# jerinphilip/whisper.tflite

Measured on AMD Instinct MI355X. Metric: audio-sec/s (RTF) whisper-tiny 30s clips batch=32 at 1/2/4/8 MI355X, higher is better.
Workload: dtype f32 (operands as two fp16 planes, f16 MFMA, f32 accumulate); 1 GPU; whisper-tiny batch=32x30s synthetic mel U(-1,1.5), fp32, random-init weights (BASELINE.json configs[1]); mel resident in HBM -> token ids on host; clips_per_gpu=32, global_batch=32, decoder_positions=30, argmax_steps=27, parallelism=clip-parallel dp1, one RCCL all_gather of id records per 8 batches, pipelined=True, batches_in_flight=10, decoder=2 consecutive steps' batches share one decoder chain (dec_pair, dec_group), last_batches_announced=2, priming_batches=1

## Files before the change

whisper.tflite_amd/csrc/k_gemm_planes.hip:

```cpp
#include <hip/hip_runtime.h>

#include <algorithm>
#include <cstdlib>
#include <cstring>
#include <type_traits>

#include "bf16_split.h"
#include "kernels.h"

namespace wt {

static int g_plane_gemm_mode = -1;
int plane_gemm_mode() {
  if (g_plane_gemm_mode < 0) {
    const char* v = getenv("WT_PLANE_GEMM_MODE");
    g_plane_gemm_mode = v ? atoi(v) : 2;
  }
  return g_plane_gemm_mode;
}
void set_plane_gemm_mode(int m) { g_plane_gemm_mode = m; }

namespace {

using f32x16 = __attribute__((ext_vector_type(16))) float;
using f32x4 = __attribute__((ext_vector_type(4))) float;
using half8 = __attribute__((ext_vector_type(8))) _Float16;
using half4 = __attribute__((ext_vector_type(4))) _Float16;
using u32x4 = __attribute__((ext_vector_type(4))) unsigned;

constexpr int BK = 32;

struct PlaneGemmDev {
  const _Float16* A;
  long a_plane;
  const _Float16* W;
  float* C;
  _Float16* P;
  long p_plane;
  const float* bias;
  const float* R;
  const float* pos;
  int M, N, K;
  int a_rpb;
  long a_bs;
  int lda;
  int c_rpb;
  long c_bs;
  int ldc;
  int pos_period;
  int kv_batch, kv_heads, kv_dmodel;
  float descale;
  float out_scale[3];
  int seg;
  const float* ln_g;
  const float* ln_b;
  _Float16* ln_P;
  long ln_plane;
  float ln_scale;
  float* ln_y32;
  int* nonfinite;
};

__host__ __device__ __forceinline__ constexpr int chunk_swizzle(int row) { return (0 - (row >> 2)) & 3; }

template <int QA, int QW, int NW, int QPW>
__device__ __forceinline__ void setup_stage_dma(const PlaneGemmDev& g, int m0, int n0, int wid, int lane, unsigned (&voff)[QPW],
                                                const unsigned char* (&ubase)[QPW], unsigned (&kstep)[QPW]) {
  const int srow = lane >> 2;
  const int nkt = g.K / BK;
#pragma unroll
  for (int j = 0; j < QPW; ++j) {
    const int q = wid + NW * j;
    if (q < 2 * QA) {
      const bool lo = q >= QA;
      const int row = 16 * (lo ? q - QA : q) + srow;
      const int chunk = (lane & 3) ^ chunk_swizzle(row);
      int m = m0 + row;
      m = m < g.M ? m : g.M - 1;
      voff[j] = (unsigned)(2 * ((lo ? g.a_plane : 0) + (long)(m / g.a_rpb) * g.a_bs + (long)(m % g.a_rpb) * g.lda + chunk * 8));
      ubase[j] = reinterpret_cast<const unsigned char*>(g.A);
      kstep[j] = BK * 2;
    } else {
      const int wq = q - 2 * QA;
      const int rg = wq % QW, plane = wq / QW;
      voff[j] = (unsigned)(lane * 16);
      ubase[j] = reinterpret_cast<const unsigned char*>(g.W) + ((size_t)(n0 / 16 + rg) * nkt * 2 + plane) * 1024;
      kstep[j] = 2048;
    }
  }
}

template <int MI_, int NI_>
struct Acc32 {
  static constexpr int MI = MI_, NI = NI_;
  f32x16 t[MI_][NI_];
  __device__ __forceinline__ void zero() {
#pragma unroll
    for (int i = 0; i < MI_; ++i)
#pragma unroll
      for (int j = 0; j < NI_; ++j)
#pragma unroll
        for (int r = 0; r < 16; ++r) t[i][j][r] = 0.0f;
  }
  __device__ __forceinline__ float get(int mi, int ni, int i) const { return t[mi][ni][i]; }
  __device__ __forceinline__ void set(int mi, int ni, int i, float v) { t[mi][ni][i] = v; }
  __device__ __forceinline__ void stage_write(int mi, int ni, float* stage, int lane, float scale) const {
    const int l31 = lane & 31, lh = lane >> 5;
#pragma unroll
    for (int r = 0; r < 16; ++r) stage[((r & 3) + 8 * (r >> 2) + 4 * lh) * 32 + (l31 ^ (lh * 20))] = t[mi][ni][r] * scale;
  }
};
template <int MI_, int NI_>
struct Acc16 {
  static constexpr int MI = MI_, NI = NI_;
  f32x4 t[2 * MI_][2 * NI_];
  __device__ __forceinline__ void zero() {
#pragma unroll
    for (int i = 0; i < 2 * MI_; ++i)
#pragma unroll
      for (int j = 0; j < 2 * NI_; ++j)
#pragma unroll
        for (int r = 0; r < 4; ++r) t[i][j][r] = 0.0f;
  }
  __device__ __forceinline__ float get(int mi, int ni, int i) const { return t[2 * mi + (i >> 3)][2 * ni + ((i >> 2) & 1)][i & 3]; }
  __device__ __forceinline__ void set(int mi, int ni, int i, float v) { t[2 * mi + (i >> 3)][2 * ni + ((i >> 2) & 1)][i & 3] = v; }
  __device__ __forceinline__ void stage_write(int mi, int ni, float* stage, int lane, float scale) const {
    const int c = lane & 15, q = lane >> 4;
#pragma unroll
    for (int a = 0; a < 2; ++a)
#pragma unroll
      for (int b = 0; b < 2; ++b)
#pragma unroll
        for (int r = 0; r < 4; ++r)
          stage[(16 * a + 4 * q + r) * 32 + ((16 * b + c) ^ ((q & 1) * 20))] = t[2 * mi + a][2 * ni + b][r] * scale;
  }
};

struct NoEpilogueHook {
  static constexpr bool active = false;
  __device__ __forceinline__ void operator()() const {}
};
template <class F>
struct ActiveEpilogueHook {
  static constexpr bool active = true;
  F& f;
  __device__ __forceinline__ void operator()() const { f(); }
};
template <int EPI, bool PLANES_OUT, int WN, bool LN, class Acc, class Hook = NoEpilogueHook>
__device__ __forceinline__ void planes_epilogue(const PlaneGemmDev& g, Acc& acc, unsigned char* smem, int m0, int n0, int wid, int wm,
                                                int wn, int lane, Hook hook = Hook{}) {
  constexpr int MI = Acc::MI, NI = Acc::NI;
  constexpr int BN = WN * NI * 32, NW = 2 * WN, BM = 64 * MI;
  __syncthreads();

  constexpr int SLD = 32;
  float* const stage = reinterpret_cast<float*>(smem) + wid * (32 * SLD);
  constexpr int CPL = PLANES_OUT ? 8 : 4;
  constexpr int LPR = 32 / CPL;
  constexpr int RPS = 64 / LPR;
  const int prow = lane / LPR, c0 = (lane % LPR) * CPL;
  float bias_all[NI][CPL];
#pragma unroll
  for (int ni = 0; ni < NI; ++ni)
#pragma unroll
    for (int e = 0; e < CPL; ++e) bias_all[ni][e] = (EPI & kEpiBias) ? g.bias[n0 + (wn * NI + ni) * 32 + c0 + e] : 0.0f;
  if constexpr (Hook::active) {
#pragma unroll
    for (int ni = 0; ni < NI; ++ni)
#pragma unroll
      for (int e = 0; e < CPL; e += 4)
        asm volatile("" : "+v"(bias_all[ni][e]), "+v"(bias_all[ni][e + 1]), "+v"(bias_all[ni][e + 2]), "+v"(bias_all[ni][e + 3]));
    hook();
  }
#pragma unroll
  for (int ni = 0; ni < NI; ++ni) {
    const int n = n0 + (wn * NI + ni) * 32 + c0;
    float bias_v[CPL];
#pragma unroll
    for (int e = 0; e < CPL; ++e) bias_v[e] = bias_all[ni][e];
    const float oscale = PLANES_OUT ? g.out_scale[n / g.seg] : 1.0f;
    const int slab = (EPI & kEpiKvLayout) ? n / g.kv_dmodel : 0, rem = (EPI & kEpiKvLayout) ? n % g.kv_dmodel : 0;
    const int head = rem >> 6, dd = rem & 63;
#pragma unroll
    for (int mi = 0; mi < MI; ++mi) {
      acc.stage_write(mi, ni, stage, lane, g.descale);
      const int mbase = m0 + wm * (32 * MI) + mi * 32;
      const int mb0 = mbase / g.c_rpb, mt0 = mbase % g.c_rpb;
      const int mp0 = (EPI & kEpiPos) ? mbase % g.pos_period : 0;
#pragma unroll
      for (int p = 0; p < 32 / RPS; ++p) {
        const int row = p * RPS + prow;
        float v[CPL];
#pragma unroll
        for (int e = 0; e < CPL; e += 4) {
          const f32x4 t = *reinterpret_cast<const f32x4*>(&stage[row * SLD + ((c0 + e) ^ (((row >> 2) & 1) * 20))]);
          v[e] = t[0], v[e + 1] = t[1], v[e + 2] = t[2], v[e + 3] = t[3];
        }
        if (mbase + row < g.M) {
          int mb = mb0, mt = mt0 + row;
          if (mt >= g.c_rpb) mt -= g.c_rpb, mb += 1;
#pragma unroll
          for (int e = 0; e < CPL; e += 2) {
            v[e] += bias_v[e];
            v[e + 1] += bias_v[e + 1];
            if (EPI & kEpiGelu) {
              const f32x2_t gl = gelu_erf2(f32x2_t{v[e], v[e + 1]});
              v[e] = gl[0];
              v[e + 1] = gl[1];
            }
          }
          if (EPI & kEpiPos) {
            int mp = mp0 + row;
            if (mp >= g.pos_period) mp -= g.pos_period;
#pragma unroll
            for (int e = 0; e < CPL; e += 4) {
              const f32x4 t = *reinterpret_cast<const f32x4*>(g.pos + (long)mp * g.N + n + e);
              v[e] += t[0], v[e + 1] += t[1], v[e + 2] += t[2], v[e + 3] += t[3];
            }
          }
          if (PLANES_OUT) {
            const long o = (long)mb * g.c_bs + (long)mt * g.ldc + n;
            u32x4 hi, lo;
#pragma unroll
            for (int e = 0; e < CPL; e += 2) {
              unsigned h, l;
              split_f16x2(v[e] * oscale, v[e + 1] * oscale, &h, &l);
              hi[e / 2] = h;
              lo[e / 2] = l;
            }
            *reinterpret_cast<u32x4*>(g.P + o) = hi;
            *reinterpret_cast<u32x4*>(g.P + g.p_plane + o) = lo;
          } else if (EPI & kEpiKvLayout) {
            const long o = (((long)slab * g.kv_batch + mb) * g.kv_heads + head) * (long)g.c_rpb * 64 + (long)mt * 64 + dd;
            __builtin_nontemporal_store(f32x4{v[0], v[1], v[2], v[3]}, reinterpret_cast<f32x4*>(g.C + o));
          } else if constexpr ((EPI & kEpiPower) != 0) {
            using f32x2 = __attribute__((ext_vector_type(2))) float;
            const long o = (long)mb * g.c_bs + (long)mt * g.ldc + (n >> 1);
            *reinterpret_cast<f32x2*>(g.C + o) = f32x2{v[0] * v[0] + v[1] * v[1], v[2] * v[2] + v[3] * v[3]};
          } else {
            const long o = (long)mb * g.c_bs + (long)mt * g.ldc + n;
            f32x4 out = {v[0], v[1], v[2], v[3]};
            if (EPI & kEpiResidual) out += *reinterpret_cast<const f32x4*>(g.R + o);
            *reinterpret_cast<f32x4*>(g.C + o) = out;
            if constexpr (LN) {
#pragma unroll
              for (int e = 0; e < 4; ++e) acc.set(mi, ni, 4 * p + e, out[e]);
            }
          }
        } else if constexpr (LN) {
#pragma unroll
          for (int e = 0; e < 4; ++e) acc.set(mi, ni, 4 * p + e, 0.0f);
        }
      }
    }
  }
  if constexpr (LN) {
    float* const part = reinterpret_cast<float*>(smem) + NW * (32 * SLD);
    const int rbase = wm * (32 * MI) + prow;
    float mean[MI][4], rstd[MI][4];
#pragma unroll
    for (int pass = 0; pass < 2; ++pass) {
#pragma unroll
      for (int mi = 0; mi < MI; ++mi)
#pragma unroll
        for (int p = 0; p < 4; ++p) {
          float t = 0.0f;
#pragma unroll
          for (int ni = 0; ni < NI; ++ni)
#pragma unroll
            for (int e = 0; e < 4; ++e) {
              const float x = acc.get(mi, ni, 4 * p + e) - (pass ? mean[mi][p] : 0.0f);
              t += pass ? x * x : x;
            }
          t += __shfl_xor(t, 1, 64);
          t += __shfl_xor(t, 2, 64);
          t += __shfl_xor(t, 4, 64);
          if ((lane & 7) == 0) part[pass * (BM * 4) + (rbase + mi * 32 + p * 8) * 4 + wn] = t;
        }
      __syncthreads();
#pragma unroll
      for (int mi = 0; mi < MI; ++mi)
#pragma unroll
        for (int p = 0; p < 4; ++p) {
          const f32x4 q = *reinterpret_cast<const f32x4*>(&part[pass * (BM * 4) + (rbase + mi * 32 + p * 8) * 4]);
          const float tot = ((q[0] + q[1]) + (q[2] + q[3])) * (1.0f / (float)BN);
          if (pass == 0) {
            mean[mi][p] = tot;
          } else {
            if (g.nonfinite != nullptr && (lane & 7) == 0 && wn == 0 && !(fabsf(mean[mi][p]) <= 3.0e38f && tot <= 3.0e38f)) atomicOr(g.nonfinite, 1);
            rstd[mi][p] = rsqrtf(tot + 1e-5f);
          }
        }
    }
#pragma unroll
    for (int ni = 0; ni < NI; ++ni) {
      const int n = n0 + (wn * NI + ni) * 32 + c0;
      const f32x4 gg = *reinterpret_cast<const f32x4*>(g.ln_g + n), bb = *reinterpret_cast<const f32x4*>(g.ln_b + n);
#pragma unroll
      for (int mi = 0; mi < MI; ++mi)
#pragma unroll
        for (int p = 0; p < 4; ++p) {
          const int m = m0 + rbase + mi * 32 + p * 8;
          if (m >= g.M) continue;
          f32x4 y;
#pragma unroll
          for (int e = 0; e < 4; ++e) y[e] = (acc.get(mi, ni, 4 * p + e) - mean[mi][p]) * rstd[mi][p] * gg[e] + bb[e];
          const long o = (long)m * BN + n;
          if (g.ln_y32 != nullptr) __builtin_nontemporal_store(y, reinterpret_cast<f32x4*>(g.ln_y32 + o));
          unsigned h0, l0, h1, l1;
          split_f16x2(y[0] * g.ln_scale, y[1] * g.ln_scale, &h0, &l0);
          split_f16x2(y[2] * g.ln_scale, y[3] * g.ln_scale, &h1, &l1);
          using u32x2 = __attribute__((ext_vector_type(2))) unsigned;
          *reinterpret_cast<u32x2*>(g.ln_P + o) = u32x2{h0, h1};
          *reinterpret_cast<u32x2*>(g.ln_P + g.ln_plane + o) = u32x2{l0, l1};
        }
    }
  }
}

template <int EPI, bool PLANES_OUT, int WN, int NI, int MI, bool LN = false>
__global__ __launch_bounds__(128 * WN, WN == 2 ? 2 : 2) void gemm_planes_tile(PlaneGemmDev g) {
  static_assert(!LN || (!PLANES_OUT && WN == 4 && NI == 3), "LayerNorm fusion: fp32 output, 384-column tile");
  constexpr int BN = WN * NI * 32, NW = 2 * WN, BM = 64 * MI;
  constexpr int kAPlane = BM * BK * 2, kWPlane = BN * BK * 2;
  constexpr int kStage = 2 * kAPlane + 2 * kWPlane;
  constexpr int QA = BM / 16, QW = BN / 16;
  constexpr int QT = 2 * QA + 2 * QW, QPW = QT / NW;
  static_assert(QT % NW == 0, "whole instructions per wavefront");
  extern __shared__ __attribute__((aligned(16))) unsigned char smem[];

  const int nb = gridDim.x, bid = blockIdx.x;
  const int q8 = nb >> 3, r8 = nb & 7, xcd = bid & 7;
  const int logical = (xcd < r8 ? xcd * (q8 + 1) : r8 * (q8 + 1) + (xcd - r8) * q8) + (bid >> 3);
  const int n_tiles = g.N / BN;
  const int m0 = (logical / n_tiles) * BM;
  const int n0 = (logical % n_tiles) * BN;

  const int tid = threadIdx.x;
  const int lane = tid & 63, wid = __builtin_amdgcn_readfirstlane(tid >> 6);
  const int wm = wid / WN, wn = wid % WN;
  const int l31 = lane & 31, lh = lane >> 5;

  unsigned voff[QPW], kstep[QPW];
  const unsigned char* ubase[QPW];
  const unsigned lds_base = (unsigned)(size_t)(const __attribute__((address_space(3))) unsigned char*)smem;
  setup_stage_dma<QA, QW, NW, QPW>(g, m0, n0, wid, lane, voff, ubase, kstep);
  auto issue_stage = [&](int kt, int buf) {
#pragma unroll
    for (int j = 0; j < QPW; ++j) {
      const unsigned long long sb = reinterpret_cast<unsigned long long>(ubase[j]) + (size_t)kt * kstep[j];
      const unsigned dst = lds_base + (unsigned)(buf * kStage + (wid + NW * j) * 1024);
      lds_dma16_sgpr(voff[j], sb, dst);
    }
  };

  Acc32<MI, NI> accs;
  accs.zero();
  auto& acc = accs.t;

  const int swz = chunk_swizzle(l31);
  const int a_off = (wm * (32 * MI) + l31) * 64, b_off = 2 * kAPlane + (wn * NI * 32 + l31) * 64;
  auto compute = [&](int buf) {
    const unsigned char* base = smem + buf * kStage;
#pragma unroll
    for (int ks = 0; ks < BK / 16; ++ks) {
      const int slot = ((ks * 2 + lh) ^ swz) * 16;
      half8 ah[MI], al[MI], bh[NI], bl[NI];
#pragma unroll
      for (int i = 0; i < MI; ++i) {
        ah[i] = *reinterpret_cast<const half8*>(base + a_off + i * 32 * 64 + slot);
        al[i] = *reinterpret_cast<const half8*>(base + kAPlane + a_off + i * 32 * 64 + slot);
      }
#pragma unroll
      for (int j = 0; j < NI; ++j) {
        bh[j] = *reinterpret_cast<const half8*>(base + b_off + j * 32 * 64 + slot);
        bl[j] = *reinterpret_cast<const half8*>(base + kWPlane + b_off + j * 32 * 64 + slot);
      }
#pragma unroll
      for (int i = 0; i < MI; ++i)
#pragma unroll
        for (int j = 0; j < NI; ++j) acc[i][j] = __builtin_amdgcn_mfma_f32_32x32x16_f16(ah[i], bl[j], acc[i][j], 0, 0, 0);
#pragma unroll
      for (int i = 0; i < MI; ++i)
#pragma unroll
        for (int j = 0; j < NI; ++j) acc[i][j] = __builtin_amdgcn_mfma_f32_32x32x16_f16(al[i], bh[j], acc[i][j], 0, 0, 0);
#pragma unroll
      for (int i = 0; i < MI; ++i)
#pragma unroll
        for (int j = 0; j < NI; ++j) acc[i][j] = __builtin_amdgcn_mfma_f32_32x32x16_f16(ah[i], bh[j], acc[i][j], 0, 0, 0);
    }
  };

  const int nkt = g.K / BK;
  issue_stage(0, 0);
  for (int kt = 0; kt < nkt; ++kt) {
    asm volatile("s_waitcnt vmcnt(0)" ::: "memory");
    __builtin_amdgcn_s_barrier();
    if (kt + 1 < nkt) issue_stage(kt + 1, (kt + 1) & 1);
    compute(kt & 1);
  }
  planes_epilogue<EPI, PLANES_OUT, WN, LN>(g, accs, smem, m0, n0, wid, wm, wn, lane);
}

#ifdef WT_PP_STAMPS
__device__ long long g_pp_stamps[1024 * 8 * 9];
#define PP_STAMP(i)                                  \
  do {                                               \
    const long long t_ = __builtin_readcyclecounter(); \
    st_[i] += t_ - tl_;                              \
    tl_ = t_;                                        \
  } while (0)
#else
#define PP_STAMP(i) \
  do {              \
  } while (0)
#endif

template <int EPI, bool PLANES_OUT, int MI, bool LN = false>
__global__ __launch_bounds__(512, 2) void gemm_planes_pp(PlaneGemmDev g) {
  constexpr int WN = 4, NI = 3;
  static_assert(!LN || !PLANES_OUT, "LayerNorm fusion: fp32 output");
  constexpr int BN = WN * NI * 32, NW = 2 * WN, BM = 64 * MI;
  constexpr int kAPlane = BM * BK * 2, kWPlane = BN * BK * 2;
  constexpr int kStage = 2 * kAPlane + 2 * kWPlane;
  constexpr int QA = BM / 16, QW = BN / 16;
  constexpr int QT = 2 * QA + 2 * QW, QPW = QT / NW;
  static_assert(QT % NW == 0, "whole instructions per wavefront");
#ifdef WT_PP_STAMPS
  const long long t_kernel_ = __builtin_readcyclecounter();
  const long long r_kernel_ = (long long)__builtin_amdgcn_s_memrealtime();
#endif
  extern __shared__ __attribute__((aligned(16))) unsigned char smem[];

  const int nb = gridDim.x, bid = blockIdx.x;
  const int q8 = nb >> 3, r8 = nb & 7, xcd = bid & 7;
  const int logical = (xcd < r8 ? xcd * (q8 + 1) : r8 * (q8 + 1) + (xcd - r8) * q8) + (bid >> 3);
  const int n_tiles = g.N / BN;
  const int m0 = (logical / n_tiles) * BM;
  const int n0 = (logical % n_tiles) * BN;

  const int tid = threadIdx.x;
  const int lane = tid & 63, wid = __builtin_amdgcn_readfirstlane(tid >> 6);
  const int wm = wid / WN, wn = wid % WN;
  const int l31 = lane & 31, lh = lane >> 5;

  unsigned voff[QPW], kstep[QPW];
  const unsigned char* ubase[QPW];
  const unsigned lds_base = (unsigned)(size_t)(const __attribute__((address_space(3))) unsigned char*)smem;
  setup_stage_dma<QA, QW, NW, QPW>(g, m0, n0, wid, lane, voff, ubase, kstep);
  auto issue_stage = [&](int kt, int buf) {
#pragma unroll
    for (int j = 0; j < QPW; ++j) {
      const unsigned long long sb = reinterpret_cast<unsigned long long>(ubase[j]) + (size_t)kt * kstep[j];
      const unsigned dst = lds_base + (unsigned)(buf * kStage + (wid + NW * j) * 1024);
      lds_dma16_sgpr(voff[j], sb, dst);
    }
  };

  Acc32<MI, NI> accs;
  accs.zero();
  auto& acc = accs.t;

  const int swz = chunk_swizzle(l31);
  const int a_off = (wm * (32 * MI) + l31) * 64, b_off = 2 * kAPlane + (wn * NI * 32 + l31) * 64;
  half8 ah[MI], al[MI], bh[NI], bl[NI];
  auto load_frags = [&](int buf, int ks) {
    const unsigned char* base = smem + buf * kStage;
    const int slot = ((ks * 2 + lh) ^ swz) * 16;
#pragma unroll
    for (int i = 0; i < MI; ++i) {
      ah[i] = *reinterpret_cast<const half8*>(base + a_off + i * 32 * 64 + slot);
      al[i] = *reinterpret_cast<const half8*>(base + kAPlane + a_off + i * 32 * 64 + slot);
    }
#pragma unroll
    for (int j = 0; j < NI; ++j) {
      bh[j] = *reinterpret_cast<const half8*>(base + b_off + j * 32 * 64 + slot);
      bl[j] = *reinterpret_cast<const half8*>(base + kWPlane + b_off + j * 32 * 64 + slot);
    }
  };
  auto compute = [&]() {
#pragma unroll
    for (int i = 0; i < MI; ++i)
#pragma unroll
      for (int j = 0; j < NI; ++j) acc[i][j] = __builtin_amdgcn_mfma_f32_32x32x16_f16(ah[i], bl[j], acc[i][j], 0, 0, 0);
#pragma unroll
    for (int i = 0; i < MI; ++i)
#pragma unroll
      for (int j = 0; j < NI; ++j) acc[i][j] = __builtin_amdgcn_mfma_f32_32x32x16_f16(al[i], bh[j], acc[i][j], 0, 0, 0);
#pragma unroll
    for (int i = 0; i < MI; ++i)
#pragma unroll
      for (int j = 0; j < NI; ++j) acc[i][j] = __builtin_amdgcn_mfma_f32_32x32x16_f16(ah[i], bh[j], acc[i][j], 0, 0, 0);
  };
  auto phase_end = [&]() {
    __builtin_amdgcn_sched_barrier(0);
    __builtin_amdgcn_s_barrier();
    __builtin_amdgcn_sched_barrier(0);
  };
  auto reads_done = [&]() { asm volatile("s_waitcnt lgkmcnt(0)" ::: "memory"); };
  auto dma_done = [&]() { asm volatile("s_waitcnt vmcnt(0)" ::: "memory"); };

  const int nkt = g.K / BK;
  issue_stage(0, 0);
  if (nkt > 1) {
    issue_stage(1, 1);
    asm volatile("s_waitcnt vmcnt(%0)" ::"n"(QPW) : "memory");
  } else {
    dma_done();
  }
  phase_end();
  if (wm == 1) phase_end();
  load_frags(0, 0);
  reads_done();
  phase_end();
#ifdef WT_PP_STAMPS
  long long st_[9] = {0, 0, 0, 0, 0, 0, 0, 0, 0};
  long long tl_ = __builtin_readcyclecounter();
  const long long t_begin_ = tl_;
  st_[5] = tl_ - t_kernel_;
#endif
  for (int kt = 0; kt < nkt; ++kt) {
    compute();
    phase_end();
    PP_STAMP(0);
    load_frags(kt & 1, 1);
    reads_done();
    if (wm == 1) dma_done();
    phase_end();
    PP_STAMP(1);
    compute();
    if (wm == 0) dma_done();
    phase_end();
    PP_STAMP(2);
    if (kt + 1 < nkt) {
      if (kt + 2 < nkt) issue_stage(kt + 2, kt & 1);
      load_frags((kt + 1) & 1, 0);
      reads_done();
    }
    phase_end();
    PP_STAMP(3);
  }
  if (wm == 0) phase_end();
#ifdef WT_PP_STAMPS
  const long long t_loop_end_ = __builtin_readcyclecounter();
  st_[4] = t_loop_end_ - t_begin_;
#endif
  planes_epilogue<EPI, PLANES_OUT, WN, LN>(g, accs, smem, m0, n0, wid, wm, wn, lane);
#ifdef WT_PP_STAMPS
  {
    const long long t_end_ = __builtin_readcyclecounter();
    st_[6] = t_end_ - t_loop_end_;
    st_[7] = t_end_ - t_kernel_;
    st_[8] = (long long)__builtin_amdgcn_s_memrealtime() - r_kernel_;
    if (lane == 0 && blockIdx.x < 1024)
      for (int i = 0; i < 9; ++i) g_pp_stamps[(blockIdx.x * 8 + wid) * 9 + i] = st_[i];
  }
#endif
}

template <int EPI, bool PLANES_OUT, bool LN = false>
__global__ __launch_bounds__(512, 2) void gemm_planes_pp16(PlaneGemmDev g) {
  constexpr int WN = 4, NI = 3, MI = 3;
  static_assert(!LN || !PLANES_OUT, "LayerNorm fusion: fp32 output");
  constexpr int BN = WN * NI * 32, NW = 2 * WN, BM = 64 * MI;
  constexpr int kAPlane = BM * BK * 2, kWPlane = BN * BK * 2;
  constexpr int kStage = 2 * kAPlane + 2 * kWPlane;
  constexpr int QA = BM / 16, QW = BN / 16;
  constexpr int QT = 2 * QA + 2 * QW, QPW = QT / NW;
  static_assert(QT % NW == 0, "whole instructions per wavefront");
#ifdef WT_PP_STAMPS
  const long long t_kernel_ = __builtin_readcyclecounter();
  const long long r_kernel_ = (long long)__builtin_amdgcn_s_memrealtime();
#endif
  extern __shared__ __attribute__((aligned(16))) unsigned char smem[];

  const int nb = gridDim.x, bid = blockIdx.x;
  const int q8 = nb >> 3, r8 = nb & 7, xcd = bid & 7;
  const int logical = (xcd < r8 ? xcd * (q8 + 1) : r8 * (q8 + 1) + (xcd - r8) * q8) + (bid >> 3);
  const int n_tiles = g.N / BN;
  const int m0 = (logical / n_tiles) * BM;
  const int n0 = (logical % n_tiles) * BN;

  const int tid = threadIdx.x;
  const int lane = tid & 63, wid = __builtin_amdgcn_readfirstlane(tid >> 6);
  const int wm = wid / WN, wn = wid % WN;

  unsigned voff[QPW], kstep[QPW];
  const unsigned char* ubase[QPW];
  const unsigned lds_base = (unsigned)(size_t)(const __attribute__((address_space(3))) unsigned char*)smem;
  setup_stage_dma<QA, QW, NW, QPW>(g, m0, n0, wid, lane, voff, ubase, kstep);
  auto issue_stage = [&](int kt, int buf) {
#pragma unroll
    for (int j = 0; j < QPW; ++j) {
      const unsigned long long sb = reinterpret_cast<unsigned long long>(ubase[j]) + (size_t)kt * kstep[j];
      const unsigned dst = lds_base + (unsigned)(buf * kStage + (wid + NW * j) * 1024);
      lds_dma16_sgpr(voff[j], sb, dst);
    }
  };

  Acc16<MI, NI> accs;
  accs.zero();
  auto& acc = accs.t;

  const int fc = lane & 15, fq = lane >> 4;
  const int frag = fc * 64 + ((fq ^ chunk_swizzle(fc)) * 16);
  const int a_off = wm * (32 * MI) * 64 + frag, b_off = 2 * kAPlane + wn * (NI * 32) * 64 + frag;
  half8 ah[3], al[3], bh[6], bl[6];
  auto load_b = [&](int buf) {
    const unsigned char* base = smem + buf * kStage + b_off;
#pragma unroll
    for (int j = 0; j < 6; ++j) {
      bh[j] = *reinterpret_cast<const half8*>(base + j * 1024);
      bl[j] = *reinterpret_cast<const half8*>(base + kWPlane + j * 1024);
    }
  };
  auto load_a = [&](int buf, int half) {
    const unsigned char* base = smem + buf * kStage + a_off + half * 3 * 1024;
#pragma unroll
    for (int i = 0; i < 3; ++i) {
      ah[i] = *reinterpret_cast<const half8*>(base + i * 1024);
      al[i] = *reinterpret_cast<const half8*>(base + kAPlane + i * 1024);
    }
  };
  auto compute = [&](auto half_c) {
    constexpr int H = decltype(half_c)::value;
#pragma unroll
    for (int i = 0; i < 3; ++i)
#pragma unroll
      for (int j = 0; j < 6; ++j) acc[3 * H + i][j] = __builtin_amdgcn_mfma_f32_16x16x32_f16(ah[i], bl[j], acc[3 * H + i][j], 0, 0, 0);
#pragma unroll
    for (int i = 0; i < 3; ++i)
#pragma unroll
      for (int j = 0; j < 6; ++j) acc[3 * H + i][j] = __builtin_amdgcn_mfma_f32_16x16x32_f16(al[i], bh[j], acc[3 * H + i][j], 0, 0, 0);
#pragma unroll
    for (int i = 0; i < 3; ++i)
#pragma unroll
      for (int j = 0; j < 6; ++j) acc[3 * H + i][j] = __builtin_amdgcn_mfma_f32_16x16x32_f16(ah[i], bh[j], acc[3 * H + i][j], 0, 0, 0);
  };
  using H0 = std::integral_constant<int, 0>;
  using H1 = std::integral_constant<int, 1>;
  auto phase_end = [&]() {
    __builtin_amdgcn_sched_barrier(0);
    __builtin_amdgcn_s_barrier();
    __builtin_amdgcn_sched_barrier(0);
  };
  auto reads_done = [&]() { asm volatile("s_waitcnt lgkmcnt(0)" ::: "memory"); };
  auto dma_done = [&]() { asm volatile("s_waitcnt vmcnt(0)" ::: "memory"); };

  const int nkt = g.K / BK;
  issue_stage(0, 0);
  if (nkt > 1) {
    issue_stage(1, 1);
    asm volatile("s_waitcnt vmcnt(%0)" ::"n"(QPW) : "memory");
  } else {
    dma_done();
  }
  phase_end();
  if (wm == 1) phase_end();
  load_b(0);
  load_a(0, 0);
  reads_done();
  phase_end();
#ifdef WT_PP_STAMPS
  long long st_[9] = {0, 0, 0, 0, 0, 0, 0, 0, 0};
  long long tl_ = __builtin_readcyclecounter();
  const long long t_begin_ = tl_;
  st_[5] = tl_ - t_kernel_;
#endif
  for (int kt = 0; kt < nkt; ++kt) {
    compute(H0{});
    phase_end();
    PP_STAMP(0);
    load_a(kt & 1, 1);
    reads_done();
    if (wm == 1) dma_done();
    phase_end();
    PP_STAMP(1);
    compute(H1{});
    if (wm == 0) dma_done();
    phase_end();
    PP_STAMP(2);
    if (kt + 1 < nkt) {
      if (kt + 2 < nkt) issue_stage(kt + 2, kt & 1);
      load_b((kt + 1) & 1);
      load_a((kt + 1) & 1, 0);
      reads_done();
    }
    phase_end();
    PP_STAMP(3);
  }
  if (wm == 0) phase_end();
#ifdef WT_PP_STAMPS
  const long long t_loop_end_ = __builtin_readcyclecounter();
  st_[4] = t_loop_end_ - t_begin_;
#endif
  planes_epilogue<EPI, PLANES_OUT, WN, LN>(g, accs, smem, m0, n0, wid, wm, wn, lane);
#ifdef WT_PP_STAMPS
  {
    const long long t_end_ = __builtin_readcyclecounter();
    st_[6] = t_end_ - t_loop_end_;
    st_[7] = t_end_ - t_kernel_;
    st_[8] = (long long)__builtin_amdgcn_s_memrealtime() - r_kernel_;
    if (lane == 0 && blockIdx.x < 1024)
      for (int i = 0; i < 9; ++i) g_pp_stamps[(blockIdx.x * 8 + wid) * 9 + i] = st_[i];
  }
#endif
}

template <int EPI>
__global__ __launch_bounds__(512, 2) void gemm_planes_pp16_persist(PlaneGemmDev g, int total_tiles) {
  constexpr int WN = 4, NI = 3, MI = 3;
  constexpr bool PLANES_OUT = true;
  static_assert((EPI & ~(kEpiBias | kEpiGelu)) == 0, "bias / GELU epilogues with plane output");
  constexpr int BN = WN * NI * 32, NW = 2 * WN, BM = 64 * MI;
  constexpr int kAPlane = BM * BK * 2, kWPlane = BN * BK * 2;
  constexpr int kStage = 2 * kAPlane + 2 * kWPlane;
  constexpr int QA = BM / 16, QW = BN / 16;
  constexpr int QT = 2 * QA + 2 * QW, QPW = QT / NW;
  constexpr int kEpiStores = MI * NI * 4;
  extern __shared__ __attribute__((aligned(16))) unsigned char smem[];

  const int grid = gridDim.x, bid = blockIdx.x;
  const int q8 = total_tiles >> 3, r8 = total_tiles & 7;
  const int n_tiles = g.N / BN;
  const int tid = threadIdx.x;
  const int lane = tid & 63, wid = __builtin_amdgcn_readfirstlane(tid >> 6);
  const int wm = wid / WN, wn = wid % WN;

  unsigned voff[QPW], kstep[QPW];
  const unsigned char* ubase[QPW];
  const unsigned lds_base = (unsigned)(size_t)(const __attribute__((address_space(3))) unsigned char*)smem;
  int m0 = 0, n0 = 0;
  auto set_tile = [&](int vid) {
    const int xcd = vid & 7;
    const int logical = (xcd < r8 ? xcd * (q8 + 1) : r8 * (q8 + 1) + (xcd - r8) * q8) + (vid >> 3);
    m0 = (logical / n_tiles) * BM;
    n0 = (logical % n_tiles) * BN;
    setup_stage_dma<QA, QW, NW, QPW>(g, m0, n0, wid, lane, voff, ubase, kstep);
  };
  auto issue_stage = [&](int kt) {
    const int buf = (kt + 1) & 1;
#pragma unroll
    for (int j = 0; j < QPW; ++j) {
      const unsigned long long sb = reinterpret_cast<unsigned long long>(ubase[j]) + (size_t)kt * kstep[j];
      lds_dma16_sgpr(voff[j], sb, lds_base + (unsigned)(buf * kStage + (wid + NW * j) * 1024));
    }
  };

  Acc16<MI, NI> accs;
  auto& acc = accs.t;
  const int fc = lane & 15, fq = lane >> 4;
  const int frag = fc * 64 + ((fq ^ chunk_swizzle(fc)) * 16);
  const int a_off = wm * (32 * MI) * 64 + frag, b_off = 2 * kAPlane + wn * (NI * 32) * 64 + frag;
  half8 ah[3], al[3], bh[6], bl[6];
  auto load_b = [&](int kt) {
    const unsigned char* base = smem + ((kt + 1) & 1) * kStage + b_off;
#pragma unroll
    for (int j = 0; j < 6; ++j) {
      bh[j] = *reinterpret_cast<const half8*>(base + j * 1024);
      bl[j] = *reinterpret_cast<const half8*>(base + kWPlane + j * 1024);
    }
  };
  auto load_a = [&](int kt, int half) {
    const unsigned char* base = smem + ((kt + 1) & 1) * kStage + a_off + half * 3 * 1024;
#pragma unroll
    for (int i = 0; i < 3; ++i) {
      ah[i] = *reinterpret_cast<const half8*>(base + i * 1024);
      al[i] = *reinterpret_cast<const half8*>(base + kAPlane + i * 1024);
    }
  };
  auto compute = [&](auto half_c) {
    constexpr int H = decltype(half_c)::value;
#pragma unroll
    for (int i = 0; i < 3; ++i)
#pragma unroll
      for (int j = 0; j < 6; ++j) acc[3 * H + i][j] = __builtin_amdgcn_mfma_f32_16x16x32_f16(ah[i], bl[j], acc[3 * H + i][j], 0, 0, 0);
#pragma unroll
    for (int i = 0; i < 3; ++i)
#pragma unroll
      for (int j = 0; j < 6; ++j) acc[3 * H + i][j] = __builtin_amdgcn_mfma_f32_16x16x32_f16(al[i], bh[j], acc[3 * H + i][j], 0, 0, 0);
#pragma unroll
    for (int i = 0; i < 3; ++i)
#pragma unroll
      for (int j = 0; j < 6; ++j) acc[3 * H + i][j] = __builtin_amdgcn_mfma_f32_16x16x32_f16(ah[i], bh[j], acc[3 * H + i][j], 0, 0, 0);
  };
  using H0 = std::integral_constant<int, 0>;
  using H1 = std::integral_constant<int, 1>;
  auto phase_end = [&]() {
    __builtin_amdgcn_sched_barrier(0);
    __builtin_amdgcn_s_barrier();
    __builtin_amdgcn_sched_barrier(0);
  };
  auto reads_done = [&]() { asm volatile("s_waitcnt lgkmcnt(0)" ::: "memory"); };
  auto dma_done = [&]() { asm volatile("s_waitcnt vmcnt(0)" ::: "memory"); };

  const int nkt = g.K / BK;
  int vid = bid;
  set_tile(vid);
  issue_stage(0);
  issue_stage(1);
  asm volatile("s_waitcnt vmcnt(%0)" ::"n"(QPW) : "memory");
  phase_end();
  for (;;) {
    if (wm == 1) phase_end();
    accs.zero();
    load_b(0);
    load_a(0, 0);
    reads_done();
    phase_end();
    for (int kt = 0; kt < nkt; ++kt) {
      compute(H0{});
      phase_end();
      load_a(kt, 1);
      reads_done();
      if (wm == 1) dma_done();
      phase_end();
      compute(H1{});
      if (wm == 0) dma_done();
      phase_end();
      if (kt + 1 < nkt) {
        if (kt + 2 < nkt) issue_stage(kt + 2);
        load_b(kt + 1);
        load_a(kt + 1, 0);
        reads_done();
      }
      phase_end();
    }
    if (wm == 0) phase_end();
    const int m_cur = m0, n_cur = n0;
    const int next = vid + grid;
    const bool has_next = next < total_tiles;
    const bool whole = m_cur + BM <= g.M;
    auto prefetch = [&]() {
      if (has_next) {
        set_tile(next);
        issue_stage(0);
      }
    };
    planes_epilogue<EPI, PLANES_OUT, WN, false>(g, accs, smem, m_cur, n_cur, wid, wm, wn, lane, ActiveEpilogueHook<decltype(prefetch)>{prefetch});
    if (!has_next) break;
    if (whole) {
      asm volatile("s_waitcnt vmcnt(%0)" ::"n"(kEpiStores) : "memory");
    } else {
      dma_done();
    }
    phase_end();
    issue_stage(1);
    vid = next;
  }
}

template <int EPI, bool PLANES_OUT, int WN, int NI, int MI = 3, bool LN = false>
void launch_planes_shape(const PlaneGemmDev& g, hipStream_t s, int n_cu = 0) {
  constexpr int BN = WN * NI * 32, BM = 64 * MI;
  const int blocks = ((g.M + BM - 1) / BM) * (g.N / BN);
  constexpr size_t smem = 2 * (2 * BM * BK * 2 + 2 * BN * BK * 2);
  static const bool raised = [] {
    (void)hipFuncSetAttribute(reinterpret_cast<const void*>(&gemm_planes_tile<EPI, PLANES_OUT, WN, NI, MI, LN>),
                              hipFuncAttributeMaxDynamicSharedMemorySize, 160 * 1024);
    return true;
  }();
  (void)raised;
  if constexpr (WN == 4 && NI == 3 && MI == 3) {
    if constexpr (PLANES_OUT && !LN && (EPI & ~(kEpiBias | kEpiGelu)) == 0) {
      const int cu = n_cu > 0 ? n_cu : 256;
      if (plane_gemm_mode() == 2 && cu % 8 == 0 && blocks >= 2 * cu && (g.K / BK) % 2 == 0 && g.K / BK >= 4) {
        static const bool raised_p = [] {
          (void)hipFuncSetAttribute(reinterpret_cast<const void*>(&gemm_planes_pp16_persist<EPI>), hipFuncAttributeMaxDynamicSharedMemorySize,
                                    160 * 1024);
          return true;
        }();
        (void)raised_p;
        WT_LAUNCH_TIMED((gemm_planes_pp16_persist<EPI>), dim3(cu), dim3(512), smem, s, g, blocks);
        return;
      }
    }
    if (plane_gemm_mode() == 2 || plane_gemm_mode() == 4) {
      static const bool raised_pp16 = [] {
        (void)hipFuncSetAttribute(reinterpret_cast<const void*>(&gemm_planes_pp16<EPI, PLANES_OUT, LN>),
                                  hipFuncAttributeMaxDynamicSharedMemorySize, 160 * 1024);
        return true;
      }();
      (void)raised_pp16;
      WT_LAUNCH_TIMED((gemm_planes_pp16<EPI, PLANES_OUT, LN>), dim3(blocks), dim3(512), smem, s, g);
      return;
    }
    if (plane_gemm_mode() == 1) {
      static const bool raised_pp = [] {
        (void)hipFuncSetAttribute(reinterpret_cast<const void*>(&gemm_planes_pp<EPI, PLANES_OUT, MI, LN>),
                                  hipFuncAttributeMaxDynamicSharedMemorySize, 160 * 1024);
        return true;
      }();
      (void)raised_pp;
      WT_LAUNCH_TIMED((gemm_planes_pp<EPI, PLANES_OUT, MI, LN>), dim3(blocks), dim3(512), smem, s, g);
      return;
    }
  }
  WT_LAUNCH_TIMED((gemm_planes_tile<EPI, PLANES_OUT, WN, NI, MI, LN>), dim3(blocks), dim3(128 * WN), smem, s, g);
}

template <int EPI, bool PLANES_OUT>
bool launch_planes(const PlaneGemmDev& g, int n_cu, hipStream_t s) {
  static const int forced = [] {
    const char* v = getenv("WT_PLANE_TILE");
    return v ? atoi(v) : 0;
  }();
  const int cu = n_cu > 0 ? n_cu : 256;
  auto rounds = [&](long tiles) { return (tiles + cu - 1) / cu; };
  const long rt192 = (g.M + 191) / 192, rt256 = (g.M + 255) / 256;
  const bool can_wide = g.N % 384 == 0;
  const double c_wide = can_wide ? 192.0 * 3 * rounds(rt192 * (g.N / 384)) : 1e30;
  const double c_tall = can_wide ? 256.0 * 3 * 1.08 * rounds(rt256 * (g.N / 384)) : 1e30;
  const double c_narrow = 192.0 * 1.1 * rounds(rt192 * (g.N / 128));
  int pick = c_wide <= c_narrow ? (c_tall < c_wide ? 2 : 1) : (c_tall < c_narrow ? 2 : 0);
  if (forced == 128) pick = 0;
  if (forced == 384 && can_wide) pick = 1;
  if (forced == 256 && can_wide) pick = 2;
  if constexpr (!PLANES_OUT && (EPI == (kEpiBias | kEpiResidual) || EPI == (kEpiBias | kEpiGelu | kEpiPos))) {
    if (g.ln_P != nullptr && g.N == 384 && pick != 0) {
      if (pick == 2) {
        launch_planes_shape<EPI, false, 4, 3, 4, true>(g, s);
      } else {
        launch_planes_shape<EPI, false, 4, 3, 3, true>(g, s);
      }
      return true;
    }
  }
  if (pick == 2) {
    launch_planes_shape<EPI, PLANES_OUT, 4, 3, 4>(g, s);
  } else if (pick == 1) {
    launch_planes_shape<EPI, PLANES_OUT, 4, 3, 3>(g, s, n_cu);
  } else {
    launch_planes_shape<EPI, PLANES_OUT, 2, 2, 3>(g, s);
  }
  return false;
}

}

std::vector<unsigned short> split_weight_planes(const float* W, int N, int K, int Kpad, float scale) {
  if (N % 16 != 0 || Kpad % 32 != 0 || K > Kpad) throw Error(kErrInvalidArg, "split_weight_planes: N % 16, Kpad % 32");
  std::vector<unsigned short> out(size_t(2) * N * Kpad, 0);
  const int nkt = Kpad / 32;
  for (int n = 0; n < N; ++n) {
    const int rg = n / 16, r = n % 16;
    for (int k = 0; k < K; ++k) {
      const float v = W[size_t(n) * K + k] * scale;
      const _Float16 h = static_cast<_Float16>(v);
      const _Float16 l = static_cast<_Float16>(v - static_cast<float>(h));
      const int kt = k / 32, c = (k % 32) / 8, e = k % 8;
      const size_t blk = (size_t(rg) * nkt + kt) * 2 * 512;
      const size_t at = size_t(r * 4 + (c ^ chunk_swizzle(r))) * 8 + e;
      std::memcpy(out.data() + blk + at, &h, 2);
      std::memcpy(out.data() + blk + 512 + at, &l, 2);
    }
  }
  return out;
}

bool launch_gemm_planes(const PlaneGemmArgs& a, int epi, hipStream_t s) {
  PlaneGemmDev g{};
  g.A = reinterpret_cast<const _Float16*>(a.A); g.a_plane = a.a_plane;
  g.W = reinterpret_cast<const _Float16*>(a.W);
  g.C = a.C; g.P = reinterpret_cast<_Float16*>(a.P); g.p_plane = a.p_plane;
  g.bias = a.bias; g.R = a.R; g.pos = a.pos;
  g.M = a.M; g.N = a.N; g.K = a.K;
  g.a_rpb = a.a_rpb; g.a_bs = a.a_bs; g.lda = a.lda;
  g.c_rpb = a.c_rpb; g.c_bs = a.c_bs; g.ldc = a.ldc;
  g.pos_period = a.pos_period;
  g.kv_batch = a.kv_batch; g.kv_heads = a.kv_heads; g.kv_dmodel = a.kv_dmodel;
  g.descale = 1.0f / (a.a_scale * a.w_scale);
  g.out_scale[0] = a.out_scale[0]; g.out_scale[1] = a.out_scale[1]; g.out_scale[2] = a.out_scale[2];
  g.seg = a.seg > 0 ? a.seg : a.N;
  g.ln_g = a.ln_g; g.ln_b = a.ln_b; g.ln_P = reinterpret_cast<_Float16*>(a.ln_P); g.ln_plane = a.ln_plane;
  g.ln_scale = a.ln_scale; g.ln_y32 = a.ln_y32; g.nonfinite = a.nonfinite;
  if (a.ln_P && (!a.ln_g || !a.ln_b || a.P || a.c_rpb < a.M || a.ldc != a.N || !(a.ln_scale > 0.0f))) {
    throw Error(kErrInvalidArg, "plane GEMM LayerNorm fusion: needs gain and shift, fp32 output, contiguous [M][N] rows");
  }
  const bool planes = a.P != nullptr;
  if (a.N % 128 != 0 || a.K % BK != 0 || a.M < 1 || a.c_rpb < 32 || a.pos_period < (epi & kEpiPos ? 32 : 1) || a.lda % 8 != 0 ||
      a.a_bs % 8 != 0 || a.ldc % 8 != 0 || a.c_bs % 8 != 0 || (planes && (g.seg % 8 != 0 || (a.N + g.seg - 1) / g.seg > 3)) ||
      (!planes && !a.C) || !(a.a_scale > 0.0f) || !(a.w_scale > 0.0f)) {
    throw Error(kErrInvalidArg, "plane GEMM shape outside the kernel contract");
  }
  {
    const long a_span = a.a_plane + (long)((a.M - 1) / a.a_rpb) * a.a_bs + (long)std::min(a.a_rpb, a.M) * a.lda + a.K + 64;
    if (a.a_plane < 0 || a.a_bs < 0 || 2 * a_span >= (1L << 32)) {
      throw Error(kErrInvalidArg, "plane GEMM operand spans more than the 4 GiB its 32-bit offsets reach");
    }
  }
  switch (epi | (planes ? 256 : 0)) {
    case kEpiBias: return launch_planes<kEpiBias, false>(g, a.n_cu, s);
    case kEpiBias | kEpiGelu: return launch_planes<kEpiBias | kEpiGelu, false>(g, a.n_cu, s);
    case kEpiBias | kEpiResidual: return launch_planes<kEpiBias | kEpiResidual, false>(g, a.n_cu, s);
    case kEpiBias | kEpiGelu | kEpiPos: return launch_planes<kEpiBias | kEpiGelu | kEpiPos, false>(g, a.n_cu, s);
    case kEpiBias | kEpiKvLayout: return launch_planes<kEpiBias | kEpiKvLayout, false>(g, a.n_cu, s);
    case kEpiBias | kEpiPower: return launch_planes<kEpiBias | kEpiPower, false>(g, a.n_cu, s);
    case kEpiBias | 256: return launch_planes<kEpiBias, true>(g, a.n_cu, s);
    case kEpiBias | kEpiGelu | 256: return launch_planes<kEpiBias | kEpiGelu, true>(g, a.n_cu, s);
    default: throw Error(kErrInvalidArg, "unsupported plane GEMM epilogue combination");
  }
}

}
```

Measured before the change: 148,400 audio-sec/s.

## Split GEMM tail wave into short-row tiles to balance last round across CUs

Adds a short-tile variant of the pp16 plane GEMM (32/64/96 rows) and a tail-split planner. The planner runs full 192-row tiles for whole CU rounds and covers the leftover rows with smaller tiles, whose relative cost comes from a hand-tuned table. The aim is to cut wave quantization, where a partial last round of big tiles leaves most CUs idle. The tile-shape picker now uses the split cost, and the narrow-tile cost factor is retuned. This adds a second kernel launch per GEMM, and the cost table may misjudge the short kernels' efficiency.

New measurement: 148,200 audio-sec/s, median of 5. Within noise of the previous version (-0.1%).

```diff
diff --git a/whisper.tflite_amd/csrc/k_gemm_planes.hip b/whisper.tflite_amd/csrc/k_gemm_planes.hip
--- a/whisper.tflite_amd/csrc/k_gemm_planes.hip
+++ b/whisper.tflite_amd/csrc/k_gemm_planes.hip
@@ -59,6 +59,7 @@
   float ln_scale;
   float* ln_y32;
   int* nonfinite;
+  int m_base;
 };
 
 __host__ __device__ __forceinline__ constexpr int chunk_swizzle(int row) { return (0 - (row >> 2)) & 3; }
@@ -92,7 +93,7 @@
 
 template <int MI_, int NI_>
 struct Acc32 {
-  static constexpr int MI = MI_, NI = NI_;
+  static constexpr int MI = MI_, NI = NI_, ROWS = 32 * MI_;
   f32x16 t[MI_][NI_];
   __device__ __forceinline__ void zero() {
 #pragma unroll
@@ -112,7 +113,7 @@
 };
 template <int MI_, int NI_>
 struct Acc16 {
-  static constexpr int MI = MI_, NI = NI_;
+  static constexpr int MI = MI_, NI = NI_, ROWS = 32 * MI_;
   f32x4 t[2 * MI_][2 * NI_];
   __device__ __forceinline__ void zero() {
 #pragma unroll
@@ -133,6 +134,39 @@
 #pragma unroll
         for (int r = 0; r < 4; ++r)
           stage[(16 * a + 4 * q + r) * 32 + ((16 * b + c) ^ ((q & 1) * 20))] = t[2 * mi + a][2 * ni + b][r] * scale;
+  }
+};
+template <int RT>
+struct AccR {
+  static constexpr int MI = (RT + 1) / 2, NI = 3, ROWS = 16 * RT;
+  f32x4 t[RT][6];
+  __device__ __forceinline__ void zero() {
+#pragma unroll
+    for (int i = 0; i < RT; ++i)
+#pragma unroll
+      for (int j = 0; j < 6; ++j)
+#pragma unroll
+        for (int r = 0; r < 4; ++r) t[i][j][r] = 0.0f;
+  }
+  __device__ __forceinline__ float get(int mi, int ni, int i) const {
+    const int a = 2 * mi + (i >> 3);
+    return a < RT ? t[a < RT ? a : 0][2 * ni + ((i >> 2) & 1)][i & 3] : 0.0f;
+  }
+  __device__ __forceinline__ void set(int mi, int ni, int i, float v) {
+    const int a = 2 * mi + (i >> 3);
+    if (a < RT) t[a < RT ? a : 0][2 * ni + ((i >> 2) & 1)][i & 3] = v;
+  }
+  __device__ __forceinline__ void stage_write(int mi, int ni, float* stage, int lane, float scale) const {
+    const int c = lane & 15, q = lane >> 4;
+#pragma unroll
+    for (int a = 0; a < 2; ++a) {
+      if (2 * mi + a >= RT) continue;
+#pragma unroll
+      for (int b = 0; b < 2; ++b)
+#pragma unroll
+        for (int r = 0; r < 4; ++r)
+          stage[(16 * a + 4 * q + r) * 32 + ((16 * b + c) ^ ((q & 1) * 20))] = t[2 * mi + a < RT ? 2 * mi + a : 0][2 * ni + b][r] * scale;
+    }
   }
 };
 
@@ -150,7 +184,8 @@
 __device__ __forceinline__ void planes_epilogue(const PlaneGemmDev& g, Acc& acc, unsigned char* smem, int m0, int n0, int wid, int wm,
                                                 int wn, int lane, Hook hook = Hook{}) {
   constexpr int MI = Acc::MI, NI = Acc::NI;
-  constexpr int BN = WN * NI * 32, NW = 2 * WN, BM = 64 * MI;
+  constexpr int WR = Acc::ROWS;
+  constexpr int BN = WN * NI * 32, NW = 2 * WN, BM = 2 * WR;
   __syncthreads();
 
   constexpr int SLD = 32;
@@ -184,11 +219,12 @@
 #pragma unroll
     for (int mi = 0; mi < MI; ++mi) {
       acc.stage_write(mi, ni, stage, lane, g.descale);
-      const int mbase = m0 + wm * (32 * MI) + mi * 32;
+      const int mbase = m0 + wm * WR + mi * 32;
       const int mb0 = mbase / g.c_rpb, mt0 = mbase % g.c_rpb;
       const int mp0 = (EPI & kEpiPos) ? mbase % g.pos_period : 0;
 #pragma unroll
       for (int p = 0; p < 32 / RPS; ++p) {
+        if (mi * 32 + p * RPS >= WR) continue;
         const int row = p * RPS + prow;
         float v[CPL];
 #pragma unroll
@@ -256,7 +292,7 @@
   }
   if constexpr (LN) {
     float* const part = reinterpret_cast<float*>(smem) + NW * (32 * SLD);
-    const int rbase = wm * (32 * MI) + prow;
+    const int rbase = wm * WR + prow;
     float mean[MI][4], rstd[MI][4];
 #pragma unroll
     for (int pass = 0; pass < 2; ++pass) {
@@ -264,6 +300,7 @@
       for (int mi = 0; mi < MI; ++mi)
 #pragma unroll
         for (int p = 0; p < 4; ++p) {
+          if (mi * 32 + p * 8 >= WR) continue;
           float t = 0.0f;
 #pragma unroll
           for (int ni = 0; ni < NI; ++ni)
@@ -282,6 +319,7 @@
       for (int mi = 0; mi < MI; ++mi)
 #pragma unroll
         for (int p = 0; p < 4; ++p) {
+          if (mi * 32 + p * 8 >= WR) continue;
           const f32x4 q = *reinterpret_cast<const f32x4*>(&part[pass * (BM * 4) + (rbase + mi * 32 + p * 8) * 4]);
           const float tot = ((q[0] + q[1]) + (q[2] + q[3])) * (1.0f / (float)BN);
           if (pass == 0) {
@@ -301,7 +339,7 @@
 #pragma unroll
         for (int p = 0; p < 4; ++p) {
           const int m = m0 + rbase + mi * 32 + p * 8;
-          if (m >= g.M) continue;
+          if (mi * 32 + p * 8 >= WR || m >= g.M) continue;
           f32x4 y;
 #pragma unroll
           for (int e = 0; e < 4; ++e) y[e] = (acc.get(mi, ni, 4 * p + e) - mean[mi][p]) * rstd[mi][p] * gg[e] + bb[e];
@@ -850,6 +888,209 @@
   }
 }
 
+template <int EPI, bool PLANES_OUT, bool LN, int RT>
+__global__ __launch_bounds__(512, 2) void gemm_planes_pp16_short(PlaneGemmDev g) {
+  constexpr int WN = 4, NI = 3;
+  static_assert(RT >= 1 && RT <= 3, "32, 64 or 96 rows");
+  static_assert(!LN || !PLANES_OUT, "LayerNorm fusion: fp32 output");
+  constexpr int BN = WN * NI * 32, NW = 2 * WN, BM = 32 * RT;
+  constexpr int kAPlane = BM * BK * 2, kWPlane = BN * BK * 2;
+  constexpr int kStage = 2 * kAPlane + 2 * kWPlane;
+  constexpr int QA = BM / 16, QW = BN / 16;
+  constexpr int QT = 2 * QA + 2 * QW, QPW = (QT + NW - 1) / NW;
+  extern __shared__ __attribute__((aligned(16))) unsigned char smem[];
+
+  const int nb = gridDim.x, bid = blockIdx.x;
+  const int q8 = nb >> 3, r8 = nb & 7, xcd = bid & 7;
+  const int logical = (xcd < r8 ? xcd * (q8 + 1) : r8 * (q8 + 1) + (xcd - r8) * q8) + (bid >> 3);
+  const int n_tiles = g.N / BN;
+  const int m0 = g.m_base + (logical / n_tiles) * BM;
+  const int n0 = (logical % n_tiles) * BN;
+
+  const int tid = threadIdx.x;
+  const int lane = tid & 63, wid = __builtin_amdgcn_readfirstlane(tid >> 6);
+  const int wm = wid / WN, wn = wid % WN;
+
+  unsigned voff[QPW], kstep[QPW];
+  const unsigned char* ubase[QPW];
+  const unsigned lds_base = (unsigned)(size_t)(const __attribute__((address_space(3))) unsigned char*)smem;
+  setup_stage_dma<QA, QW, NW, QPW>(g, m0, n0, wid, lane, voff, ubase, kstep);
+  auto issue_stage = [&](int kt, int buf) {
+#pragma unroll
+    for (int j = 0; j < QPW; ++j) {
+      if (wid + NW * j >= QT) break;
+      const unsigned long long sb = reinterpret_cast<unsigned long long>(ubase[j]) + (size_t)kt * kstep[j];
+      const unsigned dst = lds_base + (unsigned)(buf * kStage + (wid + NW * j) * 1024);
+      lds_dma16_sgpr(voff[j], sb, dst);
+    }
+  };
+
+  AccR<RT> accs;
+  accs.zero();
+  auto& acc = accs.t;
+
+  const int fc = lane & 15, fq = lane >> 4;
+  const int frag = fc * 64 + ((fq ^ chunk_swizzle(fc)) * 16);
+  const int a_off = wm * (16 * RT) * 64 + frag, b_off = 2 * kAPlane + wn * (NI * 32) * 64 + frag;
+  half8 ah[RT], al[RT], bh[3], bl[3];
+  auto load_a = [&](int buf) {
+    const unsigned char* base = smem + buf * kStage + a_off;
+#pragma unroll
+    for (int i = 0; i < RT; ++i) {
+      ah[i] = *reinterpret_cast<const half8*>(base + i * 1024);
+      al[i] = *reinterpret_cast<const half8*>(base + kAPlane + i * 1024);
+    }
+  };
+  auto load_b = [&](int buf, int half) {
+    const unsigned char* base = smem + buf * kStage + b_off + half * 3 * 1024;
+#pragma unroll
+    for (int j = 0; j < 3; ++j) {
+      bh[j] = *reinterpret_cast<const half8*>(base + j * 1024);
+      bl[j] = *reinterpret_cast<const half8*>(base + kWPlane + j * 1024);
+    }
+  };
+  auto compute = [&](auto half_c) {
+    constexpr int H = decltype(half_c)::value;
+#pragma unroll
+    for (int i = 0; i < RT; ++i)
+#pragma unroll
+      for (int j = 0; j < 3; ++j) acc[i][3 * H + j] = __builtin_amdgcn_mfma_f32_16x16x32_f16(ah[i], bl[j], acc[i][3 * H + j], 0, 0, 0);
+#pragma unroll
+    for (int i = 0; i < RT; ++i)
+#pragma unroll
+      for (int j = 0; j < 3; ++j) acc[i][3 * H + j] = __builtin_amdgcn_mfma_f32_16x16x32_f16(al[i], bh[j], acc[i][3 * H + j], 0, 0, 0);
+#pragma unroll
+    for (int i = 0; i < RT; ++i)
+#pragma unroll
+      for (int j = 0; j < 3; ++j) acc[i][3 * H + j] = __builtin_amdgcn_mfma_f32_16x16x32_f16(ah[i], bh[j], acc[i][3 * H + j], 0, 0, 0);
+  };
+  using H0 = std::integral_constant<int, 0>;
+  using H1 = std::integral_constant<int, 1>;
+  auto phase_end = [&]() {
+    __builtin_amdgcn_sched_barrier(0);
+    __builtin_amdgcn_s_barrier();
+    __builtin_amdgcn_sched_barrier(0);
+  };
+  auto reads_done = [&]() { asm volatile("s_waitcnt lgkmcnt(0)" ::: "memory"); };
+  auto dma_done = [&]() { asm volatile("s_waitcnt vmcnt(0)" ::: "memory"); };
+
+  const int nkt = g.K / BK;
+  issue_stage(0, 0);
+  if (nkt > 1) issue_stage(1, 1);
+  dma_done();
+  phase_end();
+  if (wm == 1) phase_end();
+  load_b(0, 0);
+  load_a(0);
+  reads_done();
+  phase_end();
+  for (int kt = 0; kt < nkt; ++kt) {
+    compute(H0{});
+    phase_end();
+    load_b(kt & 1, 1);
+    reads_done();
+    if (wm == 1) dma_done();
+    phase_end();
+    compute(H1{});
+    if (wm == 0) dma_done();
+    phase_end();
+    if (kt + 1 < nkt) {
+      if (kt + 2 < nkt) issue_stage(kt + 2, kt & 1);
+      load_b((kt + 1) & 1, 0);
+      load_a((kt + 1) & 1);
+      reads_done();
+    }
+    phase_end();
+  }
+  if (wm == 0) phase_end();
+  planes_epilogue<EPI, PLANES_OUT, WN, LN>(g, accs, smem, m0, n0, wid, wm, wn, lane);
+}
+
+constexpr double kShortCost[4] = {0.0, 0.22, 0.37, 0.52};
+struct TailSplit {
+  int full_tiles = 0;
+  int m_full = 0;
+  int rt = 0;
+  int short_tiles = 0;
+  double rounds = 0;
+};
+int forced_short_rows() {
+  static const int rows = [] {
+    const char* v = getenv("WT_PLANE_SHORT");
+    return v ? atoi(v) : 0;
+  }();
+  return rows == 32 || rows == 64 || rows == 96 ? rows : 0;
+}
+TailSplit tail_split(int M, int n_tiles, int cu) {
+  const int forced_rows = forced_short_rows();
+  TailSplit t;
+  if (forced_rows > 0) {
+    t.rt = forced_rows / 32;
+    t.short_tiles = (M + forced_rows - 1) / forced_rows * n_tiles;
+    t.rounds = (double)((t.short_tiles + cu - 1) / cu) * kShortCost[t.rt];
+    return t;
+  }
+  const long tiles = (long)((M + 191) / 192) * n_tiles;
+  const long full_rounds = tiles / cu;
+  t.full_tiles = (int)tiles;
+  t.m_full = M;
+  t.rounds = (double)((tiles + cu - 1) / cu);
+  if (full_rounds == 0 || tiles % cu == 0) return t;
+  const int full_rows = (int)(full_rounds * cu / n_tiles);
+  const int m_full = full_rows * 192, left = M - m_full;
+  for (int rt = 3; rt >= 1; --rt) {
+    const long pieces = (long)((left + 32 * rt - 1) / (32 * rt)) * n_tiles;
+    const double cost = (double)((long)full_rows * n_tiles + cu - 1) / cu + (double)((pieces + cu - 1) / cu) * kShortCost[rt];
+    if (cost < t.rounds - 1e-9) {
+      t.rounds = cost;
+      t.rt = rt;
+      t.full_tiles = full_rows * n_tiles;
+      t.m_full = m_full;
+      t.short_tiles = (int)pieces;
+    }
+  }
+  return t;
+}
+
+template <int EPI, bool PLANES_OUT, bool LN, int RT>
+void launch_short(const PlaneGemmDev& g0, int m_base, int tiles, hipStream_t s) {
+  constexpr size_t smem = 2 * (2 * 32 * RT * BK * 2 + 2 * 384 * BK * 2);
+  static const bool raised = [] {
+    (void)hipFuncSetAttribute(reinterpret_cast<const void*>(&gemm_planes_pp16_short<EPI, PLANES_OUT, LN, RT>),
+                              hipFuncAttributeMaxDynamicSharedMemorySize, 160 * 1024);
+    return true;
+  }();
+  (void)raised;
+  PlaneGemmDev g = g0;
+  g.m_base = m_base;
+  WT_LAUNCH_TIMED((gemm_planes_pp16_short<EPI, PLANES_OUT, LN, RT>), dim3(tiles), dim3(512), smem, s, g);
+}
+
+template <int EPI, bool PLANES_OUT, bool LN>
+void launch_planes_pp16(const PlaneGemmDev& g, hipStream_t s, int cu, int blocks) {
+  constexpr size_t smem = 2 * (2 * 192 * BK * 2 + 2 * 384 * BK * 2);
+  if (blocks == 0) return;
+  if constexpr (PLANES_OUT && !LN && (EPI & ~(kEpiBias | kEpiGelu)) == 0) {
+    if (plane_gemm_mode() == 2 && cu % 8 == 0 && blocks >= 2 * cu && (g.K / BK) % 2 == 0 && g.K / BK >= 4) {
+      static const bool raised_p = [] {
+        (void)hipFuncSetAttribute(reinterpret_cast<const void*>(&gemm_planes_pp16_persist<EPI>), hipFuncAttributeMaxDynamicSharedMemorySize,
+                                  160 * 1024);
+        return true;
+      }();
+      (void)raised_p;
+      WT_LAUNCH_TIMED((gemm_planes_pp16_persist<EPI>), dim3(cu), dim3(512), smem, s, g, blocks);
+      return;
+    }
+  }
+  static const bool raised_pp16 = [] {
+    (void)hipFuncSetAttribute(reinterpret_cast<const void*>(&gemm_planes_pp16<EPI, PLANES_OUT, LN>),
+                              hipFuncAttributeMaxDynamicSharedMemorySize, 160 * 1024);
+    return true;
+  }();
+  (void)raised_pp16;
+  WT_LAUNCH_TIMED((gemm_planes_pp16<EPI, PLANES_OUT, LN>), dim3(blocks), dim3(512), smem, s, g);
+}
+
 template <int EPI, bool PLANES_OUT, int WN, int NI, int MI = 3, bool LN = false>
 void launch_planes_shape(const PlaneGemmDev& g, hipStream_t s, int n_cu = 0) {
   constexpr int BN = WN * NI * 32, BM = 64 * MI;
@@ -862,27 +1103,19 @@
   }();
   (void)raised;
   if constexpr (WN == 4 && NI == 3 && MI == 3) {
-    if constexpr (PLANES_OUT && !LN && (EPI & ~(kEpiBias | kEpiGelu)) == 0) {
+    if (plane_gemm_mode() == 2 || plane_gemm_mode() == 4) {
       const int cu = n_cu > 0 ? n_cu : 256;
-      if (plane_gemm_mode() == 2 && cu % 8 == 0 && blocks >= 2 * cu && (g.K / BK) % 2 == 0 && g.K / BK >= 4) {
-        static const bool raised_p = [] {
-          (void)hipFuncSetAttribute(reinterpret_cast<const void*>(&gemm_planes_pp16_persist<EPI>), hipFuncAttributeMaxDynamicSharedMemorySize,
-                                    160 * 1024);
-          return true;
-        }();
-        (void)raised_p;
-        WT_LAUNCH_TIMED((gemm_planes_pp16_persist<EPI>), dim3(cu), dim3(512), smem, s, g, blocks);
-        return;
+      TailSplit t;
+      t.full_tiles = blocks;
+      if (PLANES_OUT || forced_short_rows() > 0) t = tail_split(g.M, g.N / BN, cu);
+      launch_planes_pp16<EPI, PLANES_OUT, LN>(g, s, cu, t.full_tiles);
+      if (t.rt == 3) {
+        launch_short<EPI, PLANES_OUT, LN, 3>(g, t.m_full, t.short_tiles, s);
+      } else if (t.rt == 2) {
+        launch_short<EPI, PLANES_OUT, LN, 2>(g, t.m_full, t.short_tiles, s);
+      } else if (t.rt == 1) {
+        launch_short<EPI, PLANES_OUT, LN, 1>(g, t.m_full, t.short_tiles, s);
       }
-    }
-    if (plane_gemm_mode() == 2 || plane_gemm_mode() == 4) {
-      static const bool raised_pp16 = [] {
-        (void)hipFuncSetAttribute(reinterpret_cast<const void*>(&gemm_planes_pp16<EPI, PLANES_OUT, LN>),
-                                  hipFuncAttributeMaxDynamicSharedMemorySize, 160 * 1024);
-        return true;
-      }();
-      (void)raised_pp16;
-      WT_LAUNCH_TIMED((gemm_planes_pp16<EPI, PLANES_OUT, LN>), dim3(blocks), dim3(512), smem, s, g);
       return;
     }
     if (plane_gemm_mode() == 1) {
@@ -909,9 +1142,10 @@
   auto rounds = [&](long tiles) { return (tiles + cu - 1) / cu; };
   const long rt192 = (g.M + 191) / 192, rt256 = (g.M + 255) / 256;
   const bool can_wide = g.N % 384 == 0;
-  const double c_wide = can_wide ? 192.0 * 3 * rounds(rt192 * (g.N / 384)) : 1e30;
+  const bool split = PLANES_OUT && (plane_gemm_mode() == 2 || plane_gemm_mode() == 4);
+  const double c_wide = !can_wide ? 1e30 : 192.0 * 3 * (split ? tail_split(g.M, g.N / 384, cu).rounds : (double)rounds(rt192 * (g.N / 384)));
   const double c_tall = can_wide ? 256.0 * 3 * 1.08 * rounds(rt256 * (g.N / 384)) : 1e30;
-  const double c_narrow = 192.0 * 1.1 * rounds(rt192 * (g.N / 128));
+  const double c_narrow = 192.0 * (split ? 1.2 : 1.1) * rounds(rt192 * (g.N / 128));
   int pick = c_wide <= c_narrow ? (c_tall < c_wide ? 2 : 1) : (c_tall < c_narrow ? 2 : 0);
   if (forced == 128) pick = 0;
   if (forced == 384 && can_wide) pick = 1;
@@ -921,7 +1155,7 @@
       if (pick == 2) {
         launch_planes_shape<EPI, false, 4, 3, 4, true>(g, s);
       } else {
-        launch_planes_shape<EPI, false, 4, 3, 3, true>(g, s);
+        launch_planes_shape<EPI, false, 4, 3, 3, true>(g, s, n_cu);
       }
       return true;
     }
```
